# SerezD/gen_adversarial

Hardware: AMD Instinct MI355X
Metric: purified images/sec (attack+encode+decode) (higher is better)
Workload: dtype f32 storage; contractions as 3x bf16 MFMA (hi/lo split), fp32 accumulate; 1 GPU; configs[1]: NVAE purify + VGG-11, 64x64, PGD-Linf step (fwd + input-grad), bs 256 images/GPU x EoT 32 = 8192 defender rows per step, alphas ours_cosine_no_preprocessing_ids.yaml x0.7, assumed NVAE config (C=32, 3x8 groups, 20 latents); images_per_gpu=256, eot=32, rows_per_gpu=8192, chunk_rows=1024, streams=2, parallelism=image-sharded x1

## Files before the change

### gen_adversarial_amd/csrc/conv_epilogue.h

```cpp
#pragma once
#include "ga_common.h"

namespace ga {

__device__ __forceinline__ size_t dact_row(const ga_conv_desc& d, const size_t m, const int HoWo) {
    if (d.dact_rep <= 1) return m;
    const size_t n = m / (size_t)HoWo;
    return (n / (size_t)d.dact_rep) * (size_t)HoWo + (m - n * (size_t)HoWo);
}

__device__ __forceinline__ void epilogue4(const ga_conv_desc& d, const int m, const int co, floatx4 v, const int HoWo) {
    if (d.bias) v += *reinterpret_cast<const floatx4*>(d.bias + co);
    if ((d.flags & GA_CONV_ADDEND_PRE_DACT) && d.addend) v += *reinterpret_cast<const floatx4*>(d.addend + (size_t)m * d.ldadd + co);
    if (d.dact_x) {
        floatx4 u = *reinterpret_cast<const floatx4*>(d.dact_x + dact_row(d, (size_t)m, HoWo) * d.lddact + co);
        floatx4 ds = {1.f, 1.f, 1.f, 1.f};
        if (d.flags & GA_CONV_DACT_PRELU) {
            ds = *reinterpret_cast<const floatx4*>(d.dact_scale + co);
#pragma unroll
            for (int e = 0; e < 4; ++e) v[e] *= u[e] > 0.f ? 1.f : ds[e];
        } else {
            if (d.dact_scale) {
                ds = *reinterpret_cast<const floatx4*>(d.dact_scale + co);
                u = u * ds + *reinterpret_cast<const floatx4*>(d.dact_shift + co);
            }
#pragma unroll
            for (int e = 0; e < 4; ++e) v[e] *= act_bwd_fast(u[e], d.dact_act) * ds[e];
        }
    }
    if (d.addend && !(d.flags & GA_CONV_ADDEND_PRE_DACT)) {
        size_t am = d.addend_bcast_n ? (size_t)(m % HoWo) : (size_t)m;
        if (d.addend_rep > 1) am = (size_t)((m / HoWo) / d.addend_rep) * HoWo + (m % HoWo);
        floatx4 a = *reinterpret_cast<const floatx4*>(d.addend + am * d.ldadd + co);
        if (d.flags & GA_CONV_ADDEND_RELU) { for (int e = 0; e < 4; ++e) a[e] = fmaxf(a[e], 0.f); }
        v += a;
    }
    if (d.addend2) v += *reinterpret_cast<const floatx4*>(d.addend2 + (size_t)m * d.ldadd2 + co);
    *reinterpret_cast<floatx4*>(d.y + (size_t)m * d.ldy + co) = v;
}

__device__ __forceinline__ void epilogue1(const ga_conv_desc& d, const int m, const int co, float v, const int HoWo) {
    if (d.bias) v += d.bias[co];
    if ((d.flags & GA_CONV_ADDEND_PRE_DACT) && d.addend) v += d.addend[(size_t)m * d.ldadd + co];
    if (d.dact_x) {
        float ds = 1.f, db = 0.f;
        if (d.dact_scale) { ds = d.dact_scale[co]; db = d.dact_shift[co]; }
        if (d.flags & GA_CONV_DACT_PRELU) {
            v *= d.dact_x[dact_row(d, (size_t)m, HoWo) * d.lddact + co] > 0.f ? 1.f : ds;
        } else {
            const float u = d.dact_x[dact_row(d, (size_t)m, HoWo) * d.lddact + co] * ds + db;
            v *= act_bwd_fast(u, d.dact_act) * ds;
        }
    }
    if (d.addend && !(d.flags & GA_CONV_ADDEND_PRE_DACT)) {
        size_t am = d.addend_bcast_n ? (size_t)(m % HoWo) : (size_t)m;
        if (d.addend_rep > 1) am = (size_t)((m / HoWo) / d.addend_rep) * HoWo + (m % HoWo);
        const float a = d.addend[am * d.ldadd + co];
        v += (d.flags & GA_CONV_ADDEND_RELU) ? fmaxf(a, 0.f) : a;
    }
    if (d.addend2) v += d.addend2[(size_t)m * d.ldadd2 + co];
    d.y[(size_t)m * d.ldy + co] = v;
}


template <int TM, int TN, class F>
__device__ __forceinline__ void acc_walk(floatx16 (&acc)[TM][TN], const int lane, F&& f) {
    const int lrow = lane & 31, lh = lane >> 5;
#pragma unroll
    for (int i = 0; i < TM; ++i)
#pragma unroll
        for (int j = 0; j < TN; ++j)
#pragma unroll
            for (int r = 0; r < 16; ++r) f(i * 32 + (r & 3) + 8 * (r >> 2) + 4 * lh, j * 32 + lrow, acc[i][j][r]);
}
template <int TM2, int TN2, class F>
__device__ __forceinline__ void acc_walk(floatx4 (&acc)[TM2][TN2], const int lane, F&& f) {
    const int lc = lane & 15, lq = lane >> 4;
#pragma unroll
    for (int i = 0; i < TM2; ++i)
#pragma unroll
        for (int j = 0; j < TN2; ++j)
#pragma unroll
            for (int r = 0; r < 4; ++r) f(i * 16 + 4 * lq + r, j * 16 + lc, acc[i][j][r]);
}

template <int WM, int WN, int TM, int TN, class ACC>
__device__ __forceinline__ void conv_epilogue(const ga_conv_desc& d, ACC& acc, float* smem, const int m0,
                                              const int n0, const int M, const int vec_out, const int splits, const int split,
                                              const int tw_shift = 31, const int row_stride = 0) {
    const int tw_mask = (int)((1u << tw_shift) - 1u);
    auto mrow = [&](const int r) __attribute__((always_inline)) { return m0 + (r >> tw_shift) * row_stride + (r & tw_mask); };
    constexpr int BM = WM * TM * 32, BN = WN * TN * 32;
    constexpr int LDC = BN + 4;
    const int tid = threadIdx.x, lane = tid & 63, wave = tid >> 6;
    const int wm = wave / WN, wn = wave % WN;
    const int HoWo = d.Ho * d.Wo;
    float* ws = splits > 1 ? d.ws + (size_t)split * M * d.Cout : nullptr;
    if (vec_out) {
        float* Cs = smem;
        constexpr int QL = BN / 4;
        constexpr int ROWS = 256 / QL;
        constexpr int NB = (BM / ROWS) < 4 ? (BM / ROWS) : 4;
        constexpr int NIT = BM / (ROWS * NB);
        static_assert(NIT * ROWS * NB == BM, "whole batches");
        const int q = tid % QL, rr = tid / QL;
        const int co = n0 + 4 * q;
        const bool mine = co < d.Cout;
        floatx4 u[1][NB], a1[1][NB], a2[1][NB];
        auto issue = [&](const int set, const int rb0) __attribute__((always_inline)) {
#pragma unroll
            for (int k = 0; k < NB; ++k) {
                const int r = rb0 + k * ROWS;
                const int mr = mrow(r);
                const bool ok = mr < M;
                if (d.dact_x) {
                    const size_t m = ok ? dact_row(d, (size_t)mr, HoWo) : 0;
                    u[set][k] = *reinterpret_cast<const floatx4*>(d.dact_x + m * d.lddact + co);
                }
                if (d.addend) {
                    size_t m = ok ? (size_t)mr : 0;
                    if (d.addend_bcast_n) m = m % HoWo;
                    if (d.addend_rep > 1) m = ((m / HoWo) / d.addend_rep) * HoWo + (m % HoWo);
                    a1[set][k] = *reinterpret_cast<const floatx4*>(d.addend + m * d.ldadd + co);
                }
                if (d.addend2) {
                    const size_t m = ok ? (size_t)mr : 0;
                    a2[set][k] = *reinterpret_cast<const floatx4*>(d.addend2 + m * d.ldadd2 + co);
                }
            }
        };
        floatx4 bias4 = {0.f, 0.f, 0.f, 0.f}, ds4 = {1.f, 1.f, 1.f, 1.f}, dt4 = {0.f, 0.f, 0.f, 0.f};
        if (mine && !ws) {
            if (d.bias) bias4 = *reinterpret_cast<const floatx4*>(d.bias + co);
            if (d.dact_x && d.dact_scale) {
                ds4 = *reinterpret_cast<const floatx4*>(d.dact_scale + co);
                dt4 = *reinterpret_cast<const floatx4*>(d.dact_shift + co);
            }
        }
        acc_walk(acc, lane, [&](const int row, const int col, const float v) {
            Cs[(wm * TM * 32 + row) * LDC + wn * TN * 32 + col] = v;
        });
        __syncthreads();
        if (mine) {
#pragma unroll 1
            for (int it = 0; it < NIT; ++it) {
                const int rb0 = rr + it * ROWS * NB, set = 0;
                floatx4 v[NB];
                bool ok[NB];
                if (!ws) issue(0, rb0);
#pragma unroll
                for (int k = 0; k < NB; ++k) {
                    const int r = rb0 + k * ROWS;
                    ok[k] = mrow(r) < M;
                    v[k] = *reinterpret_cast<const floatx4*>(Cs + r * LDC + 4 * q);
                }
                if (ws) {
#pragma unroll
                    for (int k = 0; k < NB; ++k)
                        if (ok[k]) *reinterpret_cast<floatx4*>(ws + (size_t)mrow(rb0 + k * ROWS) * d.Cout + co) = v[k];
                    continue;
                }
#pragma unroll
                for (int k = 0; k < NB; ++k) {
                    floatx4 o = v[k] + bias4;
                    const bool pre = (d.flags & GA_CONV_ADDEND_PRE_DACT) != 0;
                    if (pre && d.addend) o += a1[set][k];
                    if (d.dact_x && (d.flags & GA_CONV_DACT_PRELU)) {
#pragma unroll
                        for (int e = 0; e < 4; ++e) o[e] *= u[set][k][e] > 0.f ? 1.f : ds4[e];
                    } else if (d.dact_x) {
                        const floatx4 uu = u[set][k] * ds4 + dt4;
                        if (d.dact_act == GA_ACT_SILU) {
#pragma unroll
                            for (int e = 0; e < 4; ++e) { const float sg = fast_sigmoid(uu[e]); o[e] *= sg * (1.0f + uu[e] * (1.0f - sg)) * ds4[e]; }
                        } else {
#pragma unroll
                            for (int e = 0; e < 4; ++e) o[e] *= act_bwd_fast(uu[e], d.dact_act) * ds4[e];
                        }
                    }
                    if (d.addend && !pre) {
                        if (d.flags & GA_CONV_ADDEND_RELU) {
#pragma unroll
                            for (int e = 0; e < 4; ++e) o[e] += fmaxf(a1[set][k][e], 0.f);
                        } else {
                            o += a1[set][k];
                        }
                    }
                    if (d.addend2) o += a2[set][k];
                    if (ok[k]) *reinterpret_cast<floatx4*>(d.y + (size_t)mrow(rb0 + k * ROWS) * d.ldy + co) = o;
                }
            }
        }
    } else {
        acc_walk(acc, lane, [&](const int row, const int col, const float v) {
            const int co = n0 + wn * TN * 32 + col, m = mrow(wm * TM * 32 + row);
            if (co < d.Cout && m < M) {
                if (ws) ws[(size_t)m * d.Cout + co] = v;
                else epilogue1(d, m, co, v, HoWo);
            }
        });
    }
}

}
```

### gen_adversarial_amd/csrc/conv_mfma.hip

```cpp
#include "conv_split.h"
#include "conv_epilogue.h"

namespace ga {

constexpr int BK = 32;
constexpr int LDK = 36;

template <int WM, int WN, int TM, int TN, bool VEC, int PRO, bool FAST>
__global__ void __launch_bounds__(256)
conv_mfma_kernel(const ga_conv_desc d, const int tilesN, const int M, const int Ctot, const int Ktot, const int nkc,
                 const int vec_out, const fastdiv fd_howo, const fastdiv fd_wo) {
    constexpr int BM = WM * TM * 32, BN = WN * TN * 32;
    constexpr int RA = BM / 32, RB = BN / 32;
    constexpr int LDC = BN + 4;
    extern __shared__ __attribute__((aligned(16))) float smem[];
    float* As = smem;
    float* Bs = smem + 2 * BM * LDK;

    const int bid = xcd_tile_id();
    const int m0 = (bid / tilesN) * BM;
    const int n0 = (bid % tilesN) * BN;

    const int tid = threadIdx.x, lane = tid & 63, wave = tid >> 6;
    const int wm = wave / WN, wn = wave % WN;
// ... 58 lines not shown
            const bool cval = 4 * c4 < lim;
            const int delta = (kh * d.Wi + kw) * (in_x ? d.ldx : d.ldx2) * 4;
            const int soffA = (in_x ? c0 : c0 - d.C1) * 4;
            const unsigned bit = 1u << tap;
            if (in_x) {
#pragma unroll
                for (int i = 0; i < RA; ++i) {
                    const bool valid = cval & ((maskA[i] & bit) != 0);
                    const int off = valid ? baseA[i] + delta : INV;
                    okmask |= (valid ? 1u : 0u) << i;
                    ra[i] = __builtin_bit_cast(floatx4, __builtin_amdgcn_raw_buffer_load_b128(rsrcX, off, soffA, 0));
                }
            } else {
#pragma unroll
                for (int i = 0; i < RA; ++i) {
                    const bool valid = cval & ((maskA[i] & bit) != 0);
                    const int off = valid ? baseA2[i] + delta : INV;
                    okmask |= (valid ? 1u : 0u) << i;
                    ra[i] = __builtin_bit_cast(floatx4, __builtin_amdgcn_raw_buffer_load_b128(rsrcX2, off, soffA, 0));
                }
            }
            const int soffB = (tap * Ctot + c0) * 4;
#pragma unroll
            for (int i = 0; i < RB; ++i) {
                const int off = cval ? baseB[i] : INV;
                rb[i] = __builtin_bit_cast(floatx4, __builtin_amdgcn_raw_buffer_load_b128(rsrcW, off, soffB, 0));
            }
            if (PRO == 1) {
                if (d.pro_scale) {
                    const int pc = (in_x & cval) ? c : 0;
                    rs[0] = *reinterpret_cast<const floatx4*>(d.pro_scale + pc);
                    rt[0] = *reinterpret_cast<const floatx4*>(d.pro_shift + pc);
                }
            } else if (PRO == 2) {
#pragma unroll
                for (int i = 0; i < RA; ++i) {
                    const size_t po = (in_x && ((okmask >> i) & 1u)) ? (size_t)a_n[i] * d.C1 + c : 0;
                    rs[i] = *reinterpret_cast<const floatx4*>(d.pro_scale + po);
                    rt[i] = *reinterpret_cast<const floatx4*>(d.pro_shift + po);
                }
            }
        } else if (VEC) {
            const bool first = c < d.C1;
            const bool cok = c < Ctot;
            const float* src[RA];
            const float* wsrc[RB];
#pragma unroll
            for (int i = 0; i < RA; ++i) {
                int hi = a_h0[i] + kh, wi = a_w0[i] + kw;
                bool ok = cok & (a_n[i] >= 0) & (hi >= 0) & (wi >= 0) & (((hi | wi) & sd_mask) == 0);
                hi >>= sd_shift; wi >>= sd_shift;
                ok = ok & (hi < d.Hi) & (wi < d.Wi);
                const size_t pix = ((size_t)a_n[i] * d.Hi + hi) * d.Wi + wi;
                const size_t o1 = ok ? pix * d.ldx + c : 0;
                const size_t o2 = ok ? pix * d.ldx2 + (c - d.C1) : 0;
                src[i] = (first | !ok) ? d.x + o1 : d.x2 + o2;
                okmask |= (ok ? 1u : 0u) << i;
            }
#pragma unroll
            for (int i = 0; i < RB; ++i) {
                const int co = n0 + r0 + 32 * i;
                const bool ok = (co < d.Cout) & cok;
                wsrc[i] = d.w + (ok ? (size_t)co * Ktot + (size_t)tap * Ctot + c : 0);
                okmask |= (ok ? 1u : 0u) << (16 + i);
            }
#pragma unroll
            for (int i = 0; i < RA; ++i) ra[i] = *reinterpret_cast<const floatx4*>(src[i]);
#pragma unroll
            for (int i = 0; i < RB; ++i) rb[i] = *reinterpret_cast<const floatx4*>(wsrc[i]);
            if (PRO == 1) {
                if (d.pro_scale) {
                    const int pc = first ? c : 0;
                    rs[0] = *reinterpret_cast<const floatx4*>(d.pro_scale + pc);
                    rt[0] = *reinterpret_cast<const floatx4*>(d.pro_shift + pc);
                }
            } else if (PRO == 2) {
#pragma unroll
                for (int i = 0; i < RA; ++i) {
                    const size_t po = (first && ((okmask >> i) & 1u)) ? (size_t)a_n[i] * d.C1 + c : 0;
                    rs[i] = *reinterpret_cast<const floatx4*>(d.pro_scale + po);
                    rt[i] = *reinterpret_cast<const floatx4*>(d.pro_shift + po);
                }
            }
        } else {
#pragma unroll
            for (int i = 0; i < RA; ++i) {
                floatx4 v = {0.f, 0.f, 0.f, 0.f};
                if (a_n[i] >= 0 && c < Ctot) {
                    int hi = a_h0[i] + kh, wi = a_w0[i] + kw;
                    bool ok = (hi >= 0) & (wi >= 0);
                    if (d.sd != 1) { ok = ok && (hi % d.sd == 0) && (wi % d.sd == 0); hi /= d.sd; wi /= d.sd; }
                    ok = ok && hi < d.Hi && wi < d.Wi;
                    if (ok) {
                        const size_t pix = ((size_t)a_n[i] * d.Hi + hi) * d.Wi + wi;
#pragma unroll
                        for (int e = 0; e < 4; ++e) {
                            const int ce = c + e;
                            if (ce < d.C1) {
                                float u = d.x[pix * d.ldx + ce];
                                if (d.pro_scale && (d.flags & GA_CONV_PRO_PRELU)) {
                                    u = u > 0.f ? u : u * d.pro_scale[ce];
                                } else if (d.pro_scale) {
                                    const size_t po = (d.pro_per_row ? (size_t)a_n[i] * d.C1 : 0) + ce;
                                    u = u * d.pro_scale[po] + d.pro_shift[po];
                                }
                                v[e] = act_fwd_fast(u, d.pro_act);
                            } else if (ce < Ctot) {
                                v[e] = d.x2[pix * d.ldx2 + (ce - d.C1)];
                            }
                        }
                    }
                }
                ra[i] = v;
            }
#pragma unroll
            for (int i = 0; i < RB; ++i) {
                floatx4 v = {0.f, 0.f, 0.f, 0.f};
                const int co = n0 + r0 + 32 * i;
                if (co < d.Cout && c < Ctot) {
                    const float* wp = d.w + (size_t)co * Ktot + (size_t)tap * Ctot + c;
#pragma unroll
                    for (int e = 0; e < 4; ++e) if (c + e < Ctot) v[e] = wp[e];
                }
                rb[i] = v;
            }
        }
    };

    auto finish_tile = [&](const int buf) __attribute__((always_inline)) {
        float* Ab = As + buf * BM * LDK;
        float* Bb = Bs + buf * BN * LDK;
        const floatx4 zero = {0.f, 0.f, 0.f, 0.f};
        if (FAST) {
            const bool first = cur_c < d.C1;
#pragma unroll
            for (int i = 0; i < RA; ++i) {
                floatx4 v = ra[i];
                if (PRO != 0) {
                    floatx4 pv = v;
                    if (PRO == 2) pv = pv * rs[i] + rt[i];
                    else if (d.pro_scale && (d.flags & GA_CONV_PRO_PRELU)) {
#pragma unroll
                        for (int e = 0; e < 4; ++e) pv[e] = pv[e] > 0.f ? pv[e] : pv[e] * rs[0][e];
                    } else if (d.pro_scale) pv = pv * rs[0] + rt[0];
                    if (d.pro_act == GA_ACT_SILU) {
#pragma unroll
                        for (int e = 0; e < 4; ++e) pv[e] = pv[e] * fast_sigmoid(pv[e]);
                    } else if (d.pro_act != GA_ACT_NONE) {
#pragma unroll
                        for (int e = 0; e < 4; ++e) pv[e] = act_fwd_fast(pv[e], d.pro_act);
                    }
                    v = first ? pv : v;
                    v = (okmask >> i) & 1u ? v : zero;
                }
                *reinterpret_cast<floatx4*>(Ab + (r0 + 32 * i) * LDK + 4 * c4) = v;
            }
#pragma unroll
            for (int i = 0; i < RB; ++i) *reinterpret_cast<floatx4*>(Bb + (r0 + 32 * i) * LDK + 4 * c4) = rb[i];
        } else if (VEC) {
            const bool first = cur_c < d.C1;
#pragma unroll
            for (int i = 0; i < RA; ++i) {
                floatx4 v = ra[i];
                if (PRO != 0) {
                    floatx4 pv = v;
                    if (PRO == 2) pv = pv * rs[i] + rt[i];
                    else if (d.pro_scale && (d.flags & GA_CONV_PRO_PRELU)) {
#pragma unroll
                        for (int e = 0; e < 4; ++e) pv[e] = pv[e] > 0.f ? pv[e] : pv[e] * rs[0][e];
                    } else if (d.pro_scale) pv = pv * rs[0] + rt[0];
                    if (d.pro_act == GA_ACT_SILU) {
#pragma unroll
                        for (int e = 0; e < 4; ++e) pv[e] = pv[e] * fast_sigmoid(pv[e]);
                    } else if (d.pro_act != GA_ACT_NONE) {
#pragma unroll
                        for (int e = 0; e < 4; ++e) pv[e] = act_fwd_fast(pv[e], d.pro_act);
                    }
                    v = first ? pv : v;
                }
                v = (okmask >> i) & 1u ? v : zero;
                *reinterpret_cast<floatx4*>(Ab + (r0 + 32 * i) * LDK + 4 * c4) = v;
            }
#pragma unroll
            for (int i = 0; i < RB; ++i)
                *reinterpret_cast<floatx4*>(Bb + (r0 + 32 * i) * LDK + 4 * c4) = (okmask >> (16 + i)) & 1u ? rb[i] : zero;
        } else {
#pragma unroll
            for (int i = 0; i < RA; ++i) *reinterpret_cast<floatx4*>(Ab + (r0 + 32 * i) * LDK + 4 * c4) = ra[i];
#pragma unroll
            for (int i = 0; i < RB; ++i) *reinterpret_cast<floatx4*>(Bb + (r0 + 32 * i) * LDK + 4 * c4) = rb[i];
        }
    };

    floatx16 acc[TM][TN];
#pragma unroll
    for (int i = 0; i < TM; ++i)
#pragma unroll
        for (int j = 0; j < TN; ++j)
#pragma unroll
            for (int r = 0; r < 16; ++r) acc[i][j][r] = 0.f;

    const int T = d.KH * d.KW * nkc;
    const int splits = gridDim.y, split = blockIdx.y;
    const int tper = (T + splits - 1) / splits;
    const int t_begin = split * tper;
    const int t_end = min(T, t_begin + tper);

    const int lrow = lane & 31, lh = lane >> 5;
    if (t_begin < t_end) {
        seek_tile(t_begin);
        issue_tile(t_begin);
        finish_tile(0);
    }
    __syncthreads();
    for (int t = t_begin; t < t_end; ++t) {
        const int buf = (t - t_begin) & 1;
        if (t + 1 < t_end) issue_tile(t + 1);
        const float* Ab = As + buf * BM * LDK + (wm * TM * 32 + lrow) * LDK + 4 * lh;
        const float* Bb = Bs + buf * BN * LDK + (wn * TN * 32 + lrow) * LDK + 4 * lh;
#pragma unroll
        for (int kk = 0; kk < BK / 8; ++kk) {
            floatx4 af[TM], bf[TN];
#pragma unroll
            for (int i = 0; i < TM; ++i) af[i] = *reinterpret_cast<const floatx4*>(Ab + i * 32 * LDK + kk * 8);
#pragma unroll
            for (int j = 0; j < TN; ++j) bf[j] = *reinterpret_cast<const floatx4*>(Bb + j * 32 * LDK + kk * 8);
#pragma unroll
            for (int s = 0; s < 4; ++s)
#pragma unroll
                for (int i = 0; i < TM; ++i)
#pragma unroll
                    for (int j = 0; j < TN; ++j)
                        acc[i][j] = __builtin_amdgcn_mfma_f32_32x32x2f32(af[i][s], bf[j][s], acc[i][j], 0, 0, 0);
        }
        if (t + 1 < t_end) finish_tile(buf ^ 1);
        __syncthreads();
    }

    conv_epilogue<WM, WN, TM, TN>(d, acc, smem, m0, n0, M, vec_out, splits, split);
}

__global__ void __launch_bounds__(256) conv_splitk_reduce_kernel(const ga_conv_desc d, const int M, const int splits, const int vec_out) {
    const int HoWo = d.Ho * d.Wo;
    const size_t slab = (size_t)M * d.Cout;
    if (vec_out) {
        const long total4 = (long)slab / 4;
        const int C4 = d.Cout / 4;
        for (long i = (long)blockIdx.x * 256 + threadIdx.x; i < total4; i += (long)gridDim.x * 256) {
            floatx4 v = *reinterpret_cast<const floatx4*>(d.ws + i * 4);
            for (int s = 1; s < splits; ++s) v += *reinterpret_cast<const floatx4*>(d.ws + s * slab + i * 4);
            epilogue4(d, (int)(i / C4), (int)(i % C4) * 4, v, HoWo);
        }
    } else {
        for (long i = (long)blockIdx.x * 256 + threadIdx.x; i < (long)slab; i += (long)gridDim.x * 256) {
            float v = d.ws[i];
            for (int s = 1; s < splits; ++s) v += d.ws[s * slab + i];
            epilogue1(d, (int)(i / d.Cout), (int)(i % d.Cout), v, HoWo);
        }
    }
}

template <int WM, int WN, int TM, int TN, bool VEC, int PRO, bool FAST>
static void launch_inst(const ga_conv_desc& d, hipStream_t stream, dim3 grid, size_t lds, int tilesN, int M, int Ctot,
                        int Ktot, int nkc, int vec_out) {
    static dyn_lds_cache attr;
    (void)ensure_dyn_lds(attr, reinterpret_cast<const void*>(&conv_mfma_kernel<WM, WN, TM, TN, VEC, PRO, FAST>), lds);
    hipLaunchKernelGGL((conv_mfma_kernel<WM, WN, TM, TN, VEC, PRO, FAST>), grid, dim3(256), lds, stream, d, tilesN, M, Ctot, Ktot, nkc, vec_out,
                       make_fastdiv(d.Ho * d.Wo), make_fastdiv(d.Wo));
}

template <int WM, int WN, int TM, int TN>
static int launch_conv(const ga_conv_desc& d, hipStream_t stream, bool vec, int vec_out, int splits) {
    constexpr int BM = WM * TM * 32, BN = WN * TN * 32;
    const int M = d.N * d.Ho * d.Wo;
    const int Ctot = d.C1 + d.C2;
    const int Ktot = d.KH * d.KW * Ctot;
    const int nkc = (Ctot + BK - 1) / BK;
    const int tilesM = (M + BM - 1) / BM, tilesN = (d.Cout + BN - 1) / BN;
    size_t lds = (size_t)2 * (BM + BN) * LDK * sizeof(float);
    const size_t lds_c = (size_t)BM * (BN + 4) * sizeof(float);
    if (lds_c > lds) lds = lds_c;
    const dim3 grid(tilesM * tilesN, splits);
    const int pro = d.pro_scale && d.pro_per_row ? 2 : ((d.pro_scale || d.pro_act) ? 1 : 0);
    const bool fast = vec && d.sd == 1 && (d.C2 == 0 || d.C1 % BK == 0) && d.KH * d.KW <= 32 &&
                      d.x_bytes > 0 && d.w_bytes > 0 && (d.C2 == 0 || d.x2_bytes > 0);
    if (fast) {
        if (pro == 0) launch_inst<WM, WN, TM, TN, true, 0, true>(d, stream, grid, lds, tilesN, M, Ctot, Ktot, nkc, vec_out);
        else if (pro == 1) launch_inst<WM, WN, TM, TN, true, 1, true>(d, stream, grid, lds, tilesN, M, Ctot, Ktot, nkc, vec_out);
        else launch_inst<WM, WN, TM, TN, true, 2, true>(d, stream, grid, lds, tilesN, M, Ctot, Ktot, nkc, vec_out);
    } else if (vec) {
        if (pro == 0) launch_inst<WM, WN, TM, TN, true, 0, false>(d, stream, grid, lds, tilesN, M, Ctot, Ktot, nkc, vec_out);
        else if (pro == 1) launch_inst<WM, WN, TM, TN, true, 1, false>(d, stream, grid, lds, tilesN, M, Ctot, Ktot, nkc, vec_out);
        else launch_inst<WM, WN, TM, TN, true, 2, false>(d, stream, grid, lds, tilesN, M, Ctot, Ktot, nkc, vec_out);
    } else {
        launch_inst<WM, WN, TM, TN, false, 1, false>(d, stream, grid, lds, tilesN, M, Ctot, Ktot, nkc, vec_out);
    }
    return check_launch();
}

int conv_bf3_dispatch(const ga_conv_desc& d, hipStream_t stream, int tile, int vec_out, int splits);
int conv_bf3_supports(const ga_conv_desc& d);
int conv_halo3_dispatch(const ga_conv_desc& d, hipStream_t stream, int tile, int vec_out, int splits);
int conv_halo3_supports(const ga_conv_desc& d);
int conv_thin3_dispatch(const ga_conv_desc& d, hipStream_t stream, int vec_out, int splits);
int conv_thin3_supports(const ga_conv_desc& d);
int conv_pw_frag_dispatch(const ga_conv_desc& d, hipStream_t stream, int vec_out);
int conv_pw_frag_supports(const ga_conv_desc& d, int splits);

}

static long g_conv_row_limit = 0x7fffff00L;
static long ga_conv_row_limit() { return g_conv_row_limit; }
extern "C" long ga_debug_set_conv_row_limit(long bytes) {
    const long old = g_conv_row_limit;
    g_conv_row_limit = bytes > 0 ? bytes : 0x7fffff00L;
    return old;
}

extern "C" int ga_conv2d(const ga_conv_desc* dp, void* stream_) {
    ga::clear_stale_error();
    using namespace ga;
    if (!dp) return GA_E_BADARG;
    const ga_conv_desc& d = *dp;
    hipStream_t stream = reinterpret_cast<hipStream_t>(stream_);
    if (!d.x || !d.w || !d.y) return GA_E_BADARG;
    if (d.N <= 0 || d.Hi <= 0 || d.Wi <= 0 || d.C1 <= 0 || d.C2 < 0 || d.Ho <= 0 || d.Wo <= 0 || d.Cout <= 0) return GA_E_BADARG;
    if (d.KH <= 0 || d.KW <= 0 || d.sn <= 0 || d.sd <= 0 || d.pad < 0) return GA_E_BADARG;
    if (d.sd & (d.sd - 1)) return GA_E_UNSUPPORTED;
    if (d.C2 > 0 && !d.x2) return GA_E_BADARG;
    if ((d.pro_scale == nullptr) != (d.pro_shift == nullptr)) return GA_E_BADARG;
    if (d.dact_x && ((d.dact_scale == nullptr) != (d.dact_shift == nullptr))) return GA_E_BADARG;
    if (d.ldx < d.C1 || (d.C2 > 0 && d.ldx2 < d.C2) || d.ldy < d.Cout) return GA_E_BADARG;
    if (d.addend && d.ldadd < d.Cout) return GA_E_BADARG;
    if (d.addend2 && d.ldadd2 < d.Cout) return GA_E_BADARG;
    if (d.dact_x && d.lddact < d.Cout) return GA_E_BADARG;
    if (d.dact_x && d.dact_rep > 1 && d.N % d.dact_rep) return GA_E_BADARG;
    {
        const long row_x = (long)d.Hi * d.Wi * d.ldx * 4, row_x2 = d.C2 > 0 ? (long)d.Hi * d.Wi * d.ldx2 * 4 : 0;
        long row_max = row_x > row_x2 ? row_x : row_x2;
        const long pix_out = (long)d.Ho * d.Wo * 4;
        if (pix_out * d.ldy > row_max) row_max = pix_out * d.ldy;
        if (d.addend && !d.addend_bcast_n && pix_out * d.ldadd > row_max) row_max = pix_out * d.ldadd;
        if (d.addend2 && pix_out * d.ldadd2 > row_max) row_max = pix_out * d.ldadd2;
        if (d.dact_x && pix_out * d.lddact > row_max) row_max = pix_out * d.lddact;
        const long lim = ga_conv_row_limit();
        if (d.N > 1 && row_max * d.N >= lim && row_max < lim) {
            int sub = (int)((lim - 1) / row_max);
            const int arep = d.addend && !d.addend_bcast_n && d.addend_rep > 1 ? d.addend_rep : 1;
            const int drep = d.dact_x && d.dact_rep > 1 ? d.dact_rep : 1;
            if (arep > 1 || drep > 1) {
                const long both = (long)arep * drep;
                if (d.N % arep || d.N % drep) return GA_E_BADARG;
                sub -= (int)(sub % both);
                if (sub < both) return GA_E_UNSUPPORTED;
            }
            for (int n0 = 0; n0 < d.N; n0 += sub) {
                ga_conv_desc s = d;
                s.N = d.N - n0 < sub ? d.N - n0 : sub;
                const size_t pin = (size_t)n0 * d.Hi * d.Wi, pout = (size_t)n0 * d.Ho * d.Wo;
                s.x = d.x + pin * d.ldx;
                if (d.x2) s.x2 = d.x2 + pin * d.ldx2;
                s.y = d.y + pout * d.ldy;
                if (d.addend && !d.addend_bcast_n) s.addend = d.addend + (size_t)(n0 / arep) * d.Ho * d.Wo * d.ldadd;
                if (d.addend2) s.addend2 = d.addend2 + pout * d.ldadd2;
                if (d.dact_x) s.dact_x = d.dact_x + (size_t)(n0 / drep) * d.Ho * d.Wo * d.lddact;
                if (d.pro_scale && d.pro_per_row) {
                    s.pro_scale = d.pro_scale + (size_t)n0 * d.C1;
                    s.pro_shift = d.pro_shift + (size_t)n0 * d.C1;
                }
                const int rc = ga_conv2d(&s, stream_);
                if (rc != GA_OK) return rc;
            }
            return GA_OK;
        }
    }
    if ((long)d.N * d.Ho * d.Wo > 0x7fffffffL) return GA_E_UNSUPPORTED;
    if ((long)d.KH * d.KW * (d.C1 + d.C2) > 0x7fffffffL) return GA_E_UNSUPPORTED;
    const long M = (long)d.N * d.Ho * d.Wo;
    int splits = d.splits <= 1 ? 1 : d.splits;
    if (splits > 1) {
        if (!d.ws || d.ws_floats < (long)splits * M * d.Cout) return GA_E_BADARG;
        const int T = d.KH * d.KW * ((d.C1 + d.C2 + 31) / 32);
        if (splits > T) splits = T;
        if (splits > 65535) return GA_E_UNSUPPORTED;
    }

    const bool vec = (d.C1 % 4 == 0) && (d.C2 % 4 == 0) && (d.ldx % 4 == 0) && (d.C2 == 0 || d.ldx2 % 4 == 0) &&
                     aligned16(d.x) && aligned16(d.w) && (d.C2 == 0 || aligned16(d.x2)) &&
                     (!d.pro_scale || (aligned16(d.pro_scale) && aligned16(d.pro_shift)));
    const bool vec_out = (d.Cout % 4 == 0) && (d.ldy % 4 == 0) && aligned16(d.y) && (!d.bias || aligned16(d.bias)) &&
                         (!d.addend || (d.ldadd % 4 == 0 && aligned16(d.addend))) &&
                         (!d.addend2 || (d.ldadd2 % 4 == 0 && aligned16(d.addend2))) &&
                         (!d.dact_x || (d.lddact % 4 == 0 && aligned16(d.dact_x) &&
                                        (!d.dact_scale || (aligned16(d.dact_scale) && aligned16(d.dact_shift))))) &&
                         (splits == 1 || aligned16(d.ws));

    int tile = d.tile;
    if (tile == 0) {
        if (d.Cout <= 32) tile = 4;
        else if (d.Cout <= 64) tile = (M >= 128 * 256) ? 2 : 3;
        else {
            const long b128 = ((M + 127) / 128) * ((d.Cout + 127) / 128);
            const long b12864 = ((M + 127) / 128) * ((d.Cout + 63) / 64);
            if (b128 >= 512) tile = 1;
            else if (b12864 >= 512) tile = 2;
            else tile = 3;
        }
    }
    ga_conv_desc k = d;
    const long xb = ((long)d.N * d.Hi * d.Wi - 1) * d.ldx * 4 + (long)d.C1 * 4;
    const long x2b = d.C2 > 0 ? ((long)d.N * d.Hi * d.Wi - 1) * d.ldx2 * 4 + (long)d.C2 * 4 : 0;
    const long wb = (long)d.Cout * d.KH * d.KW * (d.C1 + d.C2) * 4;
    const long lim = 0x7fffff00L;
    k.x_bytes = xb < lim ? (unsigned)xb : 0;
    k.x2_bytes = x2b < lim ? (unsigned)x2b : 0;
    k.w_bytes = wb < lim ? (unsigned)wb : 0;
    const int Ctot = d.C1 + d.C2;
    const bool bf3 = d.w_hi && d.w_lo && vec && d.sd == 1 && (d.C2 == 0 || d.C1 % 32 == 0) && (Ctot % 8 == 0) &&
                     d.KH * d.KW <= 32 && k.x_bytes > 0 && k.w_bytes > 0 && (d.C2 == 0 || k.x2_bytes > 0) &&
                     aligned16(d.w_hi) && aligned16(d.w_lo) && conv_bf3_supports(d);
    int rc;
    if (tile == 11) {
        if (!(bf3 && vec_out && conv_thin3_supports(d))) return GA_E_UNSUPPORTED;
        rc = conv_thin3_dispatch(k, stream, vec_out, splits);
    } else if (tile == 12) {
        if (!(bf3 && vec_out && conv_pw_frag_supports(d, splits))) return GA_E_UNSUPPORTED;
        rc = conv_pw_frag_dispatch(k, stream, vec_out);
    } else if (tile >= 5 && tile <= 8) {
        if (!(bf3 && vec_out && conv_halo3_supports(d))) return GA_E_UNSUPPORTED;
        rc = conv_halo3_dispatch(k, stream, tile, vec_out, splits);
    } else if (bf3) {
        rc = conv_bf3_dispatch(k, stream, tile, vec_out, splits);
    } else {
        switch (tile) {
            case 1: rc = launch_conv<2, 2, 2, 2>(k, stream, vec, vec_out, splits); break;
            case 2: rc = launch_conv<4, 1, 1, 2>(k, stream, vec, vec_out, splits); break;
            case 3: rc = launch_conv<2, 2, 1, 1>(k, stream, vec, vec_out, splits); break;
            case 4: rc = launch_conv<4, 1, 1, 1>(k, stream, vec, vec_out, splits); break;
            default: return GA_E_UNSUPPORTED;
        }
    }
    if (rc != GA_OK || splits == 1) return rc;
    long items = M * d.Cout / (vec_out ? 4 : 1);
    long blocks = (items + 255) / 256;
    if (blocks > 4096) blocks = 4096;
    hipLaunchKernelGGL(conv_splitk_reduce_kernel, dim3((unsigned)blocks), dim3(256), 0, stream, k, (int)M, splits, vec_out);
    return check_launch();
}
```

### gen_adversarial_amd/engine_core.py

```python
from __future__ import annotations

import json
import os
from typing import Callable, Dict, NamedTuple, Optional

import torch

RES_SCALE = 0.1
IMG_LD = 8
WS_FLOATS = 32 * 1024 * 1024
TUNE_FILE = os.path.join(os.path.dirname(os.path.abspath(__file__)), 'conv_tune_gfx950.json')
_TUNE_CACHE: Optional[dict] = None


def tune_cache() -> dict:
    global _TUNE_CACHE
    if _TUNE_CACHE is None:
        _TUNE_CACHE = {}
        if os.path.exists(TUNE_FILE):
            with open(TUNE_FILE) as f:
                _TUNE_CACHE = json.load(f)
    return _TUNE_CACHE


def conv_key(d) -> str:
    return ('b3_' if d.w_hi else '') + '_'.join(str(int(v)) for v in (
        d.N * d.Ho * d.Wo, d.Cout, d.C1, d.C2, d.KH, d.sn, d.sd, d.Hi, d.pro_act, bool(d.pro_scale), d.pro_per_row,
        bool(d.dact_x), d.dact_act, bool(d.addend), bool(d.addend2), d.addend_bcast_n)) + (
        f'_kw{d.KW}' if d.KW != d.KH else '')


def _ptr(t: Optional[torch.Tensor]):
    return None if t is None else t.data_ptr()


_HALO_HK, _HALO_LDH = 32, 40
_BF3_MODES = (0x000, 0x100, 0x001, 0x002, 0x003, 0x004, 0x010, 0x011, 0x020, 0x021)
_HALO_MODES = (0x00, 0x01, 0x02, 0x03, 0x04, 0x10, 0x11, 0x20)


def _a16(p) -> bool:
    return not p or p % 16 == 0


def _pro_mode(d) -> int:
    return ((2 if d.pro_per_row else 1) if d.pro_scale else 0) << 4 | d.pro_act


def _splits(d, splits=None) -> int:
    s = d.splits if splits is None else splits
    if s <= 1:
        return 1
    return min(s, d.KH * d.KW * ((d.C1 + d.C2 + 31) // 32))


def _bf3_vec_out(d, splits: int) -> bool:
    c2 = d.C2 > 0
    vec = d.C1 % 4 == 0 and d.C2 % 4 == 0 and d.ldx % 4 == 0 and (not c2 or d.ldx2 % 4 == 0) and _a16(d.x) and _a16(d.w) \
        and (not c2 or _a16(d.x2)) and (not d.pro_scale or (_a16(d.pro_scale) and _a16(d.pro_shift)))
    bf3 = bool(d.w_hi and d.w_lo) and vec and d.sd == 1 and (not c2 or d.C1 % 32 == 0) and (d.C1 + d.C2) % 8 == 0 \
        and d.KH * d.KW <= 32 and _a16(d.w_hi) and _a16(d.w_lo) and ((0x100 if c2 else 0) | _pro_mode(d)) in _BF3_MODES
    vec_out = d.Cout % 4 == 0 and d.ldy % 4 == 0 and _a16(d.y) and _a16(d.bias) \
        and (not d.addend or (d.ldadd % 4 == 0 and _a16(d.addend))) and (not d.addend2 or (d.ldadd2 % 4 == 0 and _a16(d.addend2))) \
        and (not d.dact_x or (d.lddact % 4 == 0 and _a16(d.dact_x) and (not d.dact_scale or (_a16(d.dact_scale) and _a16(d.dact_shift))))) \
        and (splits == 1 or _a16(d.ws))
    return bf3 and vec_out


def _halo_3x3(d) -> bool:
    if (d.KH, d.KW, d.sn, d.sd, d.pad, d.C2) != (3, 3, 1, 1, 1, 0) or d.Ho != d.Hi or d.Wo != d.Wi or d.C1 % _HALO_HK:
        return False
    howo = d.Ho * d.Wo
    rows = d.Wo < 128 and 128 % d.Wo == 0 and (howo % 128 == 0 or 128 % howo == 0)
    return (rows or d.Wo % 128 == 0) and _pro_mode(d) in _HALO_MODES


def _halo_geometry(d, bm: int = 128, ldh: int = _HALO_LDH):
    howo = d.Ho * d.Wo
    wide = d.Wo >= bm
    tw = bm if wide else d.Wo
    th = 1 if wide else (bm // d.Wo if howo >= bm else d.Ho)
    ni = 1 if howo >= bm else bm // howo
    ph, pw = th + 2, tw + 2

    def pad_to(nbytes, want):
        return nbytes + ((want - nbytes) % 256 + 256) % 256
    rs = pad_to(pw * ldh * 2, (tw * ldh * 2) % 256)
    is_ = pad_to(ph * rs, (th * tw * ldh * 2) % 256) // 2
    return ni, ni * ph * pw, is_


def halo_ok(d, tile: Optional[int] = None, splits: Optional[int] = None) -> bool:
    tile = d.tile if tile is None else tile
    s = _splits(d, splits)
    if tile not in (5, 6, 7) or not _bf3_vec_out(d, s) or not _halo_3x3(d):
        return False
    ni, p, is_ = _halo_geometry(d)
    if p > 13 * 32 or (p > 9 * 32 and _pro_mode(d) not in (0x00, 0x10, 0x20)) or s > d.C1 // _HALO_HK:
        return False
    bn = {5: 128, 6: 64, 7: 32}[tile]
    return (2 * ni * is_ + 2 * 2 * bn * _HALO_LDH) * 2 <= 160 * 1024


def frag_ok(d, splits: Optional[int] = None) -> bool:
    s = _splits(d, splits)
    if not d.w_frag or not _a16(d.w_frag) or not _bf3_vec_out(d, s) or not _halo_3x3(d):
        return False
    ni, p, is_ = _halo_geometry(d)
    if p > 9 * 32 or s > d.C1 // _HALO_HK:
        return False
    mode = _pro_mode(d)
    patch = 2 * ni * is_ * 2
    rp = (p * 8 + 255) >> 8
    tab = rp * 256 * 6 + (2 * (ni if mode == 0x20 else 1) * d.C1 * 4 if mode >= 0x10 else 0)
    dbuf = 2 * patch + tab <= 80 * 1024
    tab_off = ((2 if dbuf else 1) * patch + 15) // 16 * 4
    return tab_off * 4 + tab <= 80 * 1024


def thin_ok(d, splits: Optional[int] = None) -> bool:
    s = _splits(d, splits)
    if s != 1 or not d.w_frag or not _a16(d.w_frag) or not _bf3_vec_out(d, s):
        return False
    if (d.KH, d.KW, d.sn, d.sd, d.pad, d.C2) != (3, 3, 1, 1, 1, 0) or d.C1 not in (32, 64):
        return False
    return d.Ho == d.Hi and d.Wo == d.Wi and d.Ho % 8 == 0 and d.Wo % 16 == 0 and d.Wo <= 255 * 16 and _pro_mode(d) in _HALO_MODES


def pw_ok(d, splits: Optional[int] = None) -> bool:
    s = _splits(d, splits)
    if s != 1 or not _a16(d.w_frag) or not _bf3_vec_out(d, s):
        return False
    if (d.KH, d.KW, d.sn, d.sd, d.pad, d.C2) != (1, 1, 1, 1, 0, 0) or d.Ho != d.Hi or d.Wo != d.Wi:
        return False
    if d.C1 % 16 or (d.N * d.Ho * d.Wo) % 128:
        return False
    if d.N * d.Ho * d.Wo * max(d.ldx, d.ldy, d.ldadd, d.ldadd2, d.lddact) * 4 >= 0x7fffff00:
        return False
    mode = _pro_mode(d)
    return mode in (0x00, 0x01, 0x10, 0x11) or (mode == 0x20 and (d.Ho * d.Wo) % 16 == 0)


class Tile(NamedTuple):
    code: int
    bm: int
    bn: int
    ok: Callable
    split_k: Optional[str] = 'step'
    fallback: Optional[tuple] = None
    frag: Optional[Callable] = None
    weight_ok: Optional[Callable] = None


def _rows_of(d, w, taps: int) -> bool:
    return w.dim() == 2 and w.shape[1] == taps * d.C1 and d.KH * d.KW == taps and d.C2 == 0


TILES: Dict[int, Tile] = {t.code: t for t in (
    Tile(1, 128, 128, lambda d, s: True), Tile(2, 128, 64, lambda d, s: True),
    Tile(3, 64, 64, lambda d, s: True), Tile(4, 128, 32, lambda d, s: True),
    Tile(5, 128, 128, lambda d, s: halo_ok(d, 5, s), 'chunk', (0, False)),
    Tile(6, 128, 64, lambda d, s: halo_ok(d, 6, s), 'chunk', (0, False)),
    Tile(7, 128, 32, lambda d, s: halo_ok(d, 7, s), 'chunk', (0, False)),
    Tile(8, 128, 128, frag_ok, 'chunk', (5, True), lambda store, w, d: store.frag3(w),
         lambda d, w: _rows_of(d, w, 9) and d.C1 % 32 == 0),
    Tile(11, 128, 32, thin_ok, None, (7, False), lambda store, w, d: store.frag_thin(w),
         lambda d, w: _rows_of(d, w, 9) and d.C1 in (32, 64)),
    Tile(12, 128, 128, pw_ok, None, (0, False), lambda store, w, d: store.frag3(w.reshape(d.Cout, d.C1), taps=1),
         lambda d, w: w.numel() == d.Cout * d.C1 and d.C1 % 16 == 0),
)}


def resolve_tile(d, tile: int, splits: int, can_frag: Callable) -> tuple:
    while tile in TILES:
        t = TILES[tile]
        if t.fallback is None or ((t.split_k or splits <= 1) and (t.frag is None or can_frag(tile)) and t.ok(d, splits)):
            break
        tile, splits = t.fallback[0], (splits if t.fallback[1] else 1)
    return tile, splits


def candidate_tiles(d, has_weight: Callable) -> tuple:
    if not d.w_hi:
        return ()
    halo = (5, 6, 7) if (d.KH == 3 and d.KW == 3 and d.sn == 1 and d.sd == 1 and d.C2 == 0) else ()
    if halo and has_weight(8):
        halo += (8,)
    thin = (11,) if halo and has_weight(11) else ()
    pw = (12,) if has_weight(12) and (d.sn, d.sd, d.pad) == (1, 1, 0) and (d.N * d.Ho * d.Wo) % 128 == 0 else ()
    return halo + thin + pw


def tile_candidates(d, has_weight: Callable) -> list:
    M = d.N * d.Ho * d.Wo
    T = d.KH * d.KW * ((d.C1 + d.C2 + 31) // 32)
    out = []
    for use_bf3 in ((1, 0) if d.w_hi else (0,)):
        for t in [TILES[c] for c in (1, 2, 3, 4) + (candidate_tiles(d, has_weight) if use_bf3 else ())]:
            if t.bn >= 2 * max(32, d.Cout):
                continue
            blocks = -(-M // t.bm) * -(-d.Cout // t.bn)
            for splits in (1, 2, 4, 8, 16, 32):
                if splits > 1 and (t.split_k is None or blocks * splits > 2048 or T < 2 * splits or splits * M * d.Cout > WS_FLOATS):
                    continue
                if t.split_k == 'chunk' and splits > d.C1 // 32:
                    continue
                out.append((use_bf3, t.code, splits))
    return out


class WeightStore:

    def __init__(self, device):
        self.device = torch.device(device)
        self.cache: Dict[str, dict] = {}
        self.splits: Dict[int, tuple] = {}
        self.bytes = 0

    def split(self, w: torch.Tensor):
        k = w.data_ptr()
        if k not in self.splits:
            hi = w.to(torch.bfloat16)
            lo = (w - hi.float()).to(torch.bfloat16)
            self.splits[k] = (hi.contiguous(), lo.contiguous(), w)
            self.bytes += 4 * w.numel()
        return self.splits[k][0], self.splits[k][1]

    def frag3(self, w: torch.Tensor, taps: int = 9) -> torch.Tensor:
        k = ('frag3' + ('' if taps == 9 else f'_taps{taps}'), w.data_ptr())
        if k not in self.splits:
            hi, lo = self.split(w)
            cout, kk = w.shape
            c = kk // taps
            cp = (c + 31) // 32 * 32
            assert kk == taps * c and (cp == c or (taps == 1 and c % 16 == 0)), (tuple(w.shape), taps)
            nt, nkc = (cout + 127) // 128, cp // 32

            def arr(t):
                tp = torch.zeros(nt * 128, taps * cp, dtype=torch.bfloat16, device=t.device)
                tp[:cout, :kk] = t
                return tp.view(nt, 4, 32, taps, nkc, 2, 2, 8).permute(0, 4, 3, 1, 5, 6, 2, 7)
            f = torch.stack([arr(hi), arr(lo)], dim=5).contiguous()
            self.splits[k] = (f, w)
            self.bytes += 2 * f.numel()
        return self.splits[k][0]

    def frag_thin(self, w: torch.Tensor) -> torch.Tensor:
        k = ('frag_thin', w.data_ptr())
        if k not in self.splits:
            hi, lo = self.split(w)
            cout, kk = w.shape
            assert kk in (9 * 32, 9 * 64), tuple(w.shape)
            nt, ks = (cout + 31) // 32, kk // 9 // 16

            def arr(t):
                tp = torch.zeros(nt * 32, kk, dtype=torch.bfloat16, device=t.device)
                tp[:cout] = t
                return tp.view(nt, 32, 9, ks, 2, 8).permute(0, 2, 3, 4, 1, 5)
            f = torch.stack([arr(hi), arr(lo)], dim=3).contiguous()
            self.splits[k] = (f, w)
            self.bytes += 2 * f.numel()
        return self.splits[k][0]

    def get(self, key: str, fn):
        if key not in self.cache:
            d = {k: v.to(self.device, dtype=torch.float32).contiguous() for k, v in fn().items()}
            self.bytes += sum(v.numel() * 4 for v in d.values())
            self.cache[key] = d
        return self.cache[key]


class Act:

    def __init__(self, eng: "Engine", n, h, w, c, name=''):
        self.eng, self.n, self.h, self.w, self.c, self.name = eng, n, h, w, c, name
        self.t = eng.alloc((n, h, w, c))
        self._g = None
        self.g_written = False
        eng.acts[name] = self

    @property
    def g(self) -> torch.Tensor:
        if self._g is None:
            self._g = self.eng.alloc((self.n * getattr(self.eng, 'cot_rep', 1), self.h, self.w, self.c))
        return self._g
```

Before: 6400 defender rows/s (rows = images x EoT-32).

## Add quadrant-specialized 3x3 conv kernel for 4x4 maps skipping padded taps

Adds a new tile (9) for 3x3 stride-1 convolutions on 4x4 spatial inputs. Each workgroup handles one 2x2 output quadrant across 32 images, so the padded taps that fall outside the image can be skipped at compile time (25 of 36 tap-pixel MFMAs per quadrant). It stages 3x3 input patches as bf16 hi/lo in LDS with double buffering and prefetches weight fragments one step ahead. The epilogue is refactored to accept a custom row-mapping functor. The new tile becomes an autotune candidate only for matching shapes and falls back to tile 8 otherwise.

```diff
diff --git a/gen_adversarial_amd/csrc/conv_epilogue.h b/gen_adversarial_amd/csrc/conv_epilogue.h
--- a/gen_adversarial_amd/csrc/conv_epilogue.h
+++ b/gen_adversarial_amd/csrc/conv_epilogue.h
@@ -84,12 +84,9 @@
             for (int r = 0; r < 4; ++r) f(i * 16 + 4 * lq + r, j * 16 + lc, acc[i][j][r]);
 }
 
-template <int WM, int WN, int TM, int TN, class ACC>
-__device__ __forceinline__ void conv_epilogue(const ga_conv_desc& d, ACC& acc, float* smem, const int m0,
-                                              const int n0, const int M, const int vec_out, const int splits, const int split,
-                                              const int tw_shift = 31, const int row_stride = 0) {
-    const int tw_mask = (int)((1u << tw_shift) - 1u);
-    auto mrow = [&](const int r) __attribute__((always_inline)) { return m0 + (r >> tw_shift) * row_stride + (r & tw_mask); };
+template <int WM, int WN, int TM, int TN, class ACC, class MROW>
+__device__ __forceinline__ void conv_epilogue_rows(const ga_conv_desc& d, ACC& acc, float* smem, const MROW& mrow,
+                                                   const int n0, const int M, const int vec_out, const int splits, const int split) {
     constexpr int BM = WM * TM * 32, BN = WN * TN * 32;
     constexpr int LDC = BN + 4;
     const int tid = threadIdx.x, lane = tid & 63, wave = tid >> 6;
@@ -202,4 +199,13 @@
     }
 }
 
-}
+template <int WM, int WN, int TM, int TN, class ACC>
+__device__ __forceinline__ void conv_epilogue(const ga_conv_desc& d, ACC& acc, float* smem, const int m0,
+                                              const int n0, const int M, const int vec_out, const int splits, const int split,
+                                              const int tw_shift = 31, const int row_stride = 0) {
+    const int tw_mask = (int)((1u << tw_shift) - 1u);
+    auto mrow = [&](const int r) __attribute__((always_inline)) { return m0 + (r >> tw_shift) * row_stride + (r & tw_mask); };
+    conv_epilogue_rows<WM, WN, TM, TN>(d, acc, smem, mrow, n0, M, vec_out, splits, split);
+}
+
+}
diff --git a/gen_adversarial_amd/csrc/conv_mfma.hip b/gen_adversarial_amd/csrc/conv_mfma.hip
--- a/gen_adversarial_amd/csrc/conv_mfma.hip
+++ b/gen_adversarial_amd/csrc/conv_mfma.hip
@@ -384,6 +384,8 @@
 int conv_bf3_supports(const ga_conv_desc& d);
 int conv_halo3_dispatch(const ga_conv_desc& d, hipStream_t stream, int tile, int vec_out, int splits);
 int conv_halo3_supports(const ga_conv_desc& d);
+int conv_quad3_dispatch(const ga_conv_desc& d, hipStream_t stream, int vec_out, int splits);
+int conv_quad3_supports(const ga_conv_desc& d, int splits);
 int conv_thin3_dispatch(const ga_conv_desc& d, hipStream_t stream, int vec_out, int splits);
 int conv_thin3_supports(const ga_conv_desc& d);
 int conv_pw_frag_dispatch(const ga_conv_desc& d, hipStream_t stream, int vec_out);
@@ -508,6 +510,9 @@
     } else if (tile == 12) {
         if (!(bf3 && vec_out && conv_pw_frag_supports(d, splits))) return GA_E_UNSUPPORTED;
         rc = conv_pw_frag_dispatch(k, stream, vec_out);
+    } else if (tile == 9) {
+        if (!(bf3 && vec_out && conv_quad3_supports(d, splits))) return GA_E_UNSUPPORTED;
+        rc = conv_quad3_dispatch(k, stream, vec_out, splits);
     } else if (tile >= 5 && tile <= 8) {
         if (!(bf3 && vec_out && conv_halo3_supports(d))) return GA_E_UNSUPPORTED;
         rc = conv_halo3_dispatch(k, stream, tile, vec_out, splits);
diff --git a/gen_adversarial_amd/csrc/conv_quad3.hip b/gen_adversarial_amd/csrc/conv_quad3.hip
--- /dev/null
+++ b/gen_adversarial_amd/csrc/conv_quad3.hip
@@ -0,0 +1,243 @@
+#include <utility>
+#include "conv_split.h"
+#include "conv_epilogue.h"
+
+namespace ga {
+
+int conv_halo3_supports(const ga_conv_desc& d);
+
+namespace {
+
+constexpr int QK = 32;
+constexpr int QPIX = 32 * 64;
+constexpr int QPLANE = 9 * QPIX;
+constexpr int QBUF = 2 * QPLANE;
+
+constexpr int quad_pix(const int Q, const int i, const int tap) {
+    const int ry = (Q >> 1) + (i >> 1) - 1 + tap / 3, rx = (Q & 1) + (i & 1) - 1 + tap % 3;
+    return (ry >= 0 && ry <= 2 && rx >= 0 && rx <= 2) ? 3 * ry + rx : -1;
+}
+constexpr int quad_nvalid(const int Q, const int tap) {
+    int n = 0;
+    for (int i = 0; i < 4; ++i) n += quad_pix(Q, i, tap) >= 0;
+    return n;
+}
+struct quad_group { int tap, ks, i0, i1; bool first, last; };
+constexpr quad_group quad_group_at(const int Q, const int g) {
+    int n = 0;
+    for (int tap = 0; tap < 9; ++tap)
+        for (int ks = 0; ks < 2; ++ks) {
+            int v[4] = {-1, -1, -1, -1}, nv = 0;
+            for (int i = 0; i < 4; ++i)
+                if (quad_pix(Q, i, tap) >= 0) v[nv++] = i;
+            for (int k = 0; k < nv; k += 2, ++n)
+                if (n == g) return quad_group{tap, ks, v[k], k + 1 < nv ? v[k + 1] : -1, k == 0, k + 2 >= nv};
+        }
+    return quad_group{-1, 0, -1, -1, false, false};
+}
+constexpr int quad_ngroups(const int Q) {
+    int n = 0;
+    while (quad_group_at(Q, n).tap >= 0) ++n;
+    return n;
+}
+constexpr int quad_mfma3(const int Q) {
+    int n = 0;
+    for (int t = 0; t < 9; ++t) n += quad_nvalid(Q, t);
+    return n;
+}
+static_assert(quad_mfma3(0) == 25 && quad_mfma3(1) == 25 && quad_mfma3(2) == 25 && quad_mfma3(3) == 25, "4 + 6 + 6 + 9 per quadrant");
+static_assert(quad_ngroups(0) == 26 && quad_ngroups(1) == 26 && quad_ngroups(2) == 26 && quad_ngroups(3) == 26, "13 groups per k step");
+
+template <int I> using ic = std::integral_constant<int, I>;
+template <class F, int... Is>
+__device__ __forceinline__ void static_for(F&& f, std::integer_sequence<int, Is...>) { (f(ic<Is>{}), ...); }
+
+template <int AFF, int ACT>
+__global__ void __launch_bounds__(256, 2)
+conv_quad3_kernel(const ga_conv_desc d, const int tilesN, const int M, const int C, const int nkc) {
+    constexpr int WM = 1, WN = 4, TM = 4, TN = 1, BN = 128;
+    extern __shared__ __attribute__((aligned(16))) float smem[];
+    char* const sm = reinterpret_cast<char*>(smem);
+    const int bid = xcd_tile_id();
+    const int mt = bid / tilesN, nt = bid % tilesN, n0 = nt * BN;
+    const int quad = mt & 3, qy = quad >> 1, qx = quad & 1;
+    const int n_first = (mt >> 2) * 32;
+
+    const int tid = threadIdx.x, lane = tid & 63, wn = tid >> 6;
+    const int img = tid >> 3, c4 = tid & 7;
+    const int lrow = lane & 31, lh = lane >> 5;
+
+    const __amdgpu_buffer_rsrc_t rsrcX = __builtin_amdgcn_make_buffer_rsrc(const_cast<float*>(d.x), 0, d.x_bytes, 0x00020000);
+    const int pixb = d.ldx * 4;
+    const int gbase = (((n_first + img) * 4 + qy) * 4 + qx) * pixb + c4 * 16;
+    const int wbase = img * 64 + (((c4 >> 1) ^ ((img >> 2) & 3)) << 4) + ((c4 & 1) << 3);
+    const size_t prow = AFF == 2 ? (size_t)min(n_first + img, d.N - 1) * C : 0;
+    const float* const ptab_s = AFF ? d.pro_scale + prow + 4 * c4 : nullptr;
+    const float* const ptab_t = AFF ? d.pro_shift + prow + 4 * c4 : nullptr;
+    int rd[2];
+#pragma unroll
+    for (int ks = 0; ks < 2; ++ks) rd[ks] = lrow * 64 + (((2 * ks + lh) ^ ((lrow >> 2) & 3)) << 4);
+
+    const int splits = gridDim.y, split = blockIdx.y;
+    const int cper = (nkc + splits - 1) / splits;
+    const int cb = split * cper, ce = min(nkc, cb + cper);
+
+    floatx4 rpat[9], rs = {1.f, 1.f, 1.f, 1.f}, rt = {0.f, 0.f, 0.f, 0.f};
+    auto issue_patch = [&](const int chunk) __attribute__((always_inline)) {
+#pragma unroll
+        for (int j = 0; j < 9; ++j)
+            rpat[j] = __builtin_bit_cast(floatx4, __builtin_amdgcn_raw_buffer_load_b128(rsrcX, gbase, chunk * QK * 4 + ((j / 3) * 4 + j % 3) * pixb, 0));
+        if (AFF != 0) {
+            rs = *reinterpret_cast<const floatx4*>(ptab_s + chunk * QK);
+            rt = *reinterpret_cast<const floatx4*>(ptab_t + chunk * QK);
+        }
+    };
+    auto finish_patch = [&](const int buf) __attribute__((always_inline)) {
+        char* const Ph = sm + buf * QBUF + wbase;
+#pragma unroll
+        for (int j = 0; j < 9; ++j) {
+            floatx4 v = rpat[j];
+            if (AFF == 1) v = pro_affine4(v, rs, rt, d.flags & GA_CONV_PRO_PRELU);
+            if (AFF == 2) v = v * rs + rt;
+            v = pro_act4<ACT>(v);
+            if (AFF != 0) {
+#pragma unroll
+                for (int e = 0; e < 4; ++e) {
+                    float ve = v[e];
+                    asm volatile("" : "+v"(ve));
+                    v[e] = ve;
+                }
+            }
+            bf16x4 hi, lo;
+            split4(v, hi, lo);
+            *reinterpret_cast<bf16x4*>(Ph + j * QPIX) = hi;
+            *reinterpret_cast<bf16x4*>(Ph + j * QPIX + QPLANE) = lo;
+        }
+    };
+
+    const uintx4* wf = reinterpret_cast<const uintx4*>(d.w_frag) + ((size_t)nt * nkc * 9 * 4 + wn) * 4 * 64 + lane;
+    uintx4 bcur[4], bnxt[4];
+    auto load_B = [&](uintx4 (&b)[4], const int chunk, const int tap, const int ks) __attribute__((always_inline)) {
+        const uintx4* p = wf + (size_t)(chunk * 9 + tap) * (4 * 4 * 64);
+#pragma unroll
+        for (int q = 2 * ks; q < 2 * ks + 2; ++q) b[q] = p[q * 64];
+    };
+
+    floatx16 acc[TM][TN];
+#pragma unroll
+    for (int i = 0; i < TM; ++i)
+#pragma unroll
+        for (int r = 0; r < 16; ++r) acc[i][0][r] = 0.f;
+
+    if (cb < ce) {
+        issue_patch(cb);
+        load_B(bcur, cb, 0, 0);
+        load_B(bcur, cb, 0, 1);
+        finish_patch(0);
+        __builtin_amdgcn_sched_barrier(0);
+        if (cb + 1 < ce) issue_patch(cb + 1);
+    }
+    __syncthreads();
+
+    auto run = [&](auto QC) __attribute__((always_inline)) {
+        constexpr int Q = decltype(QC)::value;
+        constexpr int NG = quad_ngroups(Q);
+        bf16x8 ahs[2][2], als[2][2];
+        int buf = 0;
+#pragma unroll 1
+        for (int chunk = cb; chunk < ce; ++chunk) {
+            const char* const pa[2] = {sm + buf * QBUF + rd[0], sm + buf * QBUF + rd[1]};
+            auto load_A = [&](auto GC) __attribute__((always_inline)) {
+                constexpr int g = decltype(GC)::value;
+                constexpr quad_group G = quad_group_at(Q, g);
+#pragma unroll
+                for (int k = 0; k < 2; ++k) {
+                    const int i = k ? G.i1 : G.i0;
+                    if (i >= 0) {
+                        ahs[g & 1][k] = *reinterpret_cast<const bf16x8*>(pa[G.ks] + quad_pix(Q, i, G.tap) * QPIX);
+                        als[g & 1][k] = *reinterpret_cast<const bf16x8*>(pa[G.ks] + quad_pix(Q, i, G.tap) * QPIX + QPLANE);
+                    }
+                }
+            };
+            load_A(ic<0>{});
+            static_for([&](auto GC) __attribute__((always_inline)) {
+                constexpr int g = decltype(GC)::value;
+                constexpr quad_group G = quad_group_at(Q, g);
+                constexpr int n = G.i1 >= 0 ? 2 : 1;
+                if constexpr (G.first) {
+                    load_B(bnxt, G.tap == 8 ? min(chunk + 1, ce - 1) : chunk, G.tap == 8 ? 0 : G.tap + 1, G.ks);
+                    __builtin_amdgcn_sched_group_barrier(0x020, 2, 0);
+                }
+                if constexpr (g + 1 < NG) {
+                    load_A(ic<g + 1>{});
+                    __builtin_amdgcn_sched_group_barrier(0x100, 2 * (quad_group_at(Q, g + 1).i1 >= 0 ? 2 : 1), 0);
+                }
+                const bf16x8 bh = __builtin_bit_cast(bf16x8, bcur[2 * G.ks]), bl = __builtin_bit_cast(bf16x8, bcur[2 * G.ks + 1]);
+                mfma3(acc[G.i0][0], ahs[g & 1][0], als[g & 1][0], bh, bl);
+                if constexpr (n == 2) mfma3(acc[G.i1][0], ahs[g & 1][1], als[g & 1][1], bh, bl);
+                __builtin_amdgcn_sched_group_barrier(0x008, 3 * n, 0);
+                __builtin_amdgcn_sched_barrier(0);
+                if constexpr (g == NG / 2) {
+                    if (chunk + 1 < ce) {
+                        finish_patch(buf ^ 1);
+                        if (chunk + 2 < ce) issue_patch(chunk + 2);
+                    }
+                }
+                if constexpr (G.ks == 1 && G.last) {
+#pragma unroll
+                    for (int q = 0; q < 4; ++q) bcur[q] = bnxt[q];
+                }
+            }, std::make_integer_sequence<int, NG>{});
+            __syncthreads();
+            buf ^= 1;
+        }
+    };
+    switch (quad) {
+        case 0: run(ic<0>{}); break;
+        case 1: run(ic<1>{}); break;
+        case 2: run(ic<2>{}); break;
+        default: run(ic<3>{}); break;
+    }
+
+    const int mq = n_first * 16 + (2 * qy) * 4 + 2 * qx;
+    auto mrow = [&](const int r) __attribute__((always_inline)) { return mq + (r & 31) * 16 + ((r >> 6) << 2) + ((r >> 5) & 1); };
+    conv_epilogue_rows<WM, WN, TM, TN>(d, acc, smem, mrow, n0, M, 1, splits, split);
+}
+
+template <int AFF, int ACT>
+void launch_quad_inst(const ga_conv_desc& d, hipStream_t stream, dim3 grid, size_t lds, int tilesN, int M, int nkc) {
+    static dyn_lds_cache attr;
+    (void)ensure_dyn_lds(attr, reinterpret_cast<const void*>(&conv_quad3_kernel<AFF, ACT>), lds);
+    hipLaunchKernelGGL((conv_quad3_kernel<AFF, ACT>), grid, dim3(256), lds, stream, d, tilesN, M, d.C1, nkc);
+}
+
+}
+
+int conv_quad3_supports(const ga_conv_desc& d, const int splits) {
+    if (!conv_halo3_supports(d) || d.Hi != 4 || d.Wi != 4 || (d.N % 32 != 0 && d.N > 32)) return 0;
+    return d.w_frag && aligned16(d.w_frag) && splits <= d.C1 / QK;
+}
+
+int conv_quad3_dispatch(const ga_conv_desc& d, hipStream_t stream, int vec_out, int splits) {
+    constexpr int BM = 128, BN = 128;
+    if (!vec_out) return GA_E_UNSUPPORTED;
+    const int M = d.N * 16, nkc = d.C1 / QK;
+    const int tilesM = 4 * ((d.N + 31) / 32), tilesN = (d.Cout + BN - 1) / BN;
+    const size_t lds = 2 * QBUF;
+    static_assert(2 * QBUF >= BM * (BN + 4) * sizeof(float) && 2 * QBUF <= 80 * 1024, "two workgroups per CU");
+    const dim3 grid(tilesM * tilesN, splits);
+#define GA_QUAD(MODE, A, C, WIDE) \
+    case MODE: launch_quad_inst<A, C>(d, stream, grid, lds, tilesN, M, nkc); break;
+    switch (conv_pro_mode(d)) {
+#ifdef GA_HALO_EXP_ONLY
+        GA_CONV3_MODES_EXP(GA_QUAD)
+#else
+        GA_CONV3_MODES(GA_QUAD)
+#endif
+        default: return GA_E_UNSUPPORTED;
+    }
+#undef GA_QUAD
+    return check_launch();
+}
+
+}
diff --git a/gen_adversarial_amd/engine_core.py b/gen_adversarial_amd/engine_core.py
--- a/gen_adversarial_amd/engine_core.py
+++ b/gen_adversarial_amd/engine_core.py
@@ -118,6 +118,13 @@
     return tab_off * 4 + tab <= 80 * 1024
 
 
+def quad_ok(d, splits: Optional[int] = None) -> bool:
+    s = _splits(d, splits)
+    if not d.w_frag or not _a16(d.w_frag) or not _bf3_vec_out(d, s) or not _halo_3x3(d):
+        return False
+    return d.Hi == 4 and d.Wi == 4 and (d.N % 32 == 0 or d.N < 32) and s <= d.C1 // _HALO_HK
+
+
 def thin_ok(d, splits: Optional[int] = None) -> bool:
     s = _splits(d, splits)
     if s != 1 or not d.w_frag or not _a16(d.w_frag) or not _bf3_vec_out(d, s):
@@ -164,6 +171,8 @@
     Tile(7, 128, 32, lambda d, s: halo_ok(d, 7, s), 'chunk', (0, False)),
     Tile(8, 128, 128, frag_ok, 'chunk', (5, True), lambda store, w, d: store.frag3(w),
          lambda d, w: _rows_of(d, w, 9) and d.C1 % 32 == 0),
+    Tile(9, 128, 128, quad_ok, 'chunk', (8, True), lambda store, w, d: store.frag3(w),
+         lambda d, w: _rows_of(d, w, 9) and d.C1 % 32 == 0),
     Tile(11, 128, 32, thin_ok, None, (7, False), lambda store, w, d: store.frag_thin(w),
          lambda d, w: _rows_of(d, w, 9) and d.C1 in (32, 64)),
     Tile(12, 128, 128, pw_ok, None, (0, False), lambda store, w, d: store.frag3(w.reshape(d.Cout, d.C1), taps=1),
@@ -186,6 +195,8 @@
     halo = (5, 6, 7) if (d.KH == 3 and d.KW == 3 and d.sn == 1 and d.sd == 1 and d.C2 == 0) else ()
     if halo and has_weight(8):
         halo += (8,)
+        if d.Hi == 4 and d.Wi == 4 and (d.N % 32 == 0 or d.N < 32) and has_weight(9):
+            halo += (9,)
     thin = (11,) if halo and has_weight(11) else ()
     pw = (12,) if has_weight(12) and (d.sn, d.sd, d.pad) == (1, 1, 0) and (d.N * d.Ho * d.Wo) % 128 == 0 else ()
     return halo + thin + pw
```

Result: faster. 6587 defender rows/s (rows = images x EoT-32) (median of 6 runs) (+2.9%).
